# ElenaBiagi/Finito

Measured on AMD Instinct MI355X. Metric: localized k-mers/s (k=31), higher is better.
Workload: dtype u32

## Files before the change

### finito_amd/__init__.py

```python
import ctypes as C
import os
import subprocess

import numpy as np

_HERE = os.path.dirname(os.path.abspath(__file__))
_LIBPATH = os.path.join(_HERE, "libfinito_amd.so")
_LIB = None

FIN_FWD, FIN_MERGED = 0, 1
FIN_OK, FIN_EINVAL, FIN_EIO, FIN_ENODEV, FIN_ENOMEM, FIN_ELIMIT = 0, -1, -2, -3, -4, -5
X_C, X_PLANE_A, X_LCS, X_FMIN, X_USTART, X_GOFF, X_ENDS, X_CONCAT = 0, 1, 5, 6, 7, 8, 9, 10
DT_PTAB, DT_JTAB, DT_FILT, DT_SAFE, DT_RCWIN, DT_CBF, DT_FBF = range(7)


class FinitoError(RuntimeError):

    def __init__(self, code, msg):
        super().__init__("%s (code %d)" % (msg, code))
        self.code = code


def host_threads():
    n = len(os.sched_getaffinity(0)) if hasattr(os, "sched_getaffinity") else (os.cpu_count() or 1)
    for path in ("/sys/fs/cgroup/cpu.max", "/sys/fs/cgroup/cpu/cpu.cfs_quota_us"):
        try:
            txt = open(path).read().split()
            if path.endswith("cpu.max"):
# ... 948 lines not shown
        return bool(self.L.fin_index_is_disjoint(self.h))

    def seed_table(self, device=0):
        import numpy as np
        out = np.empty((self.n_nodes, 2), dtype=np.uint32)
        err = C.create_string_buffer(512)
        rc = self.L.fin_index_debug_seed_table(self.h, int(device), out.ctypes.data_as(C.c_void_p), err, 512)
        return out if rc == 0 else None

    def debug_table(self, what, device=0):
        nbytes = int(self.L.fin_index_debug_table_bytes(self.h, int(device), int(what)))
        if nbytes < 0:
            raise FinitoError(FIN_EINVAL, "debug_table: no replica on device %d, or no table %r" % (device, what))
        if nbytes == 0:
            return None
        dt = {DT_SAFE: np.uint64, DT_RCWIN: np.uint8}.get(what, np.uint32)
        out = np.zeros(nbytes // np.dtype(dt).itemsize, dtype=dt)
        err = C.create_string_buffer(512)
        _check(self.L.fin_index_debug_table(self.h, int(device), int(what), out.ctypes.data_as(C.c_void_p), out.nbytes, err, 512), err)
        return out.reshape(-1, 2) if what in (DT_PTAB, DT_JTAB) else out.reshape(-1, 4) if what in (DT_CBF, DT_FBF) else out

    def string_filter_geometry(self, device=0):
        m, lg = C.c_uint32(0), C.c_uint32(0)
        rc = self.L.fin_index_string_filter_geometry(self.h, int(device), C.byref(m), C.byref(lg))
        if rc != 0:
            raise FinitoError(rc, "string_filter_geometry: no replica on device %d" % device)
        return int(m.value), int(lg.value)

    def kmer_table_query(self, kmers, device=0):
        k = self.k
        code = {"A": 0, "C": 1, "G": 2, "T": 3}
        k0 = np.zeros(len(kmers), dtype=np.uint64); k1 = np.zeros(len(kmers), dtype=np.uint64)
        for i, s in enumerate(kmers):
            a = b = 0
            for j, ch in enumerate(s):
# ... 574 lines not shown
```

### finito_amd/csrc/fin_capi.cpp

```cpp
#include <functional>
#include <hip/hip_runtime_api.h>
#include <sched.h>

#include <algorithm>
#include <atomic>
#include <chrono>
#include <condition_variable>
#include <cstdio>
#include <cstdlib>
#include <cstring>
#include <memory>
#include <mutex>
#include <new>
#include <string>
#include <thread>
#include <vector>

#include "../../include/finito_amd.h"
#include "fin_index.hpp"
#include "fin_kernels.h"

static void set_err(char* err, size_t errlen, const std::string& msg) {
    if (err && errlen) { snprintf(err, errlen, "%s", msg.c_str()); }
}
// ... 46 lines not shown
StagePool g_stage;
bool is_page_locked(const void* p) {
    if (!p) return true;
    hipPointerAttribute_t a;
    memset(&a, 0, sizeof a);
    if (hipPointerGetAttributes(&a, p) != hipSuccess) { (void)hipGetLastError(); return false; }
    return a.type == hipMemoryTypeHost;
}
}

extern "C" {

const char* fin_version(void) { return "finito-amd 0.1 (gfx950)"; }

enum : int { O_lds_deque_limit, O_kernel, O_probe_prepass, O_ptab_t, O_jtab_t, O_write_gaps, O_overlap_prefill, O_filt_f, O_seed_anchors, O_kmer_table,
              O_defer_strand, O_fast_path, O_cbf_m, O_lean_tables, O_text_anchors, O_epoch_budget_mult, O_epoch_budget_add, O_max_batch_kmers, O_pipeline_kmers, O_pipeline_depth, O_stage_pageable, O_debug_ovf_cap, O_debug_pp_seg, O_lean_walk, O_fused_ingest, O_pp_park, O_debug_pp_park_cap, O_pp_wide_out, O_hits_combine, O_cover_probe, O_debug_depth_tile, O_ec_tag_bits, O_ec_combine, O_COUNT };
static_assert(O_COUNT <= FIN_N_OPTIONS, "fin_index::opt_val has room for every option");
struct OptDef { const char* name; int64_t def, lo, hi; };
static const OptDef OPTS[O_COUNT] = {
    {"lds_deque_limit", 16, 1, 16},
    {"kernel", 4, 0, 4},
    {"probe_prepass", 1, 0, 1},
    {"ptab_t", -1, -1, 15},
    {"jtab_t", -1, -1, 14},
    {"write_gaps", 1, 0, 1},
    {"overlap_prefill", 1, 0, 1},
    {"filt_f", -1, -1, 16},
    {"seed_anchors", 1, 0, 1},
    {"kmer_table", 1, 0, 1},
    {"defer_strand", 1, 0, 1},
    {"fast_path", 1, 0, 2},
// ... 1 lines not shown
    {"lean_tables", 2, 0, 3},
    {"text_anchors", 1, 0, 1},
    {"epoch_budget_mult", 64, 0, 64},
    {"epoch_budget_add", 4096, 1, 1 << 20},
    {"max_batch_kmers", 1ll << 30, 1, 1ll << 31},
    {"pipeline_kmers", 1ll << 26, 1, 1ll << 31},
    {"pipeline_depth", 3, 1, 8},
    {"stage_pageable", 1, 0, 1},
    {"debug_ovf_cap", 0, 0, 1ll << 31},
    {"debug_pp_seg", 0, 0, 1024},
    {"lean_walk", 1, 0, 1},
    {"fused_ingest", 1, 0, 1},
    {"pp_park", 1, 0, 1},
    {"debug_pp_park_cap", -1, -1, 1024},
    {"pp_wide_out", 1, 0, 1},
    {"hits_combine", 4, 0, 64},
    {"cover_probe", 0, 0, 1},
    {"debug_depth_tile", 0, 0, 4096},
    {"ec_tag_bits", 63, 1, 63},
    {"ec_combine", 1, 0, 1},
};
static std::atomic<int64_t> g_opt[O_COUNT];
static const bool g_opt_init = [] { for (int i = 0; i < O_COUNT; i++) g_opt[i].store(OPTS[i].def); return true; }();
static inline int64_t optv(const fin_index* x, int id) { return x && x->opt_set[id].load(std::memory_order_acquire) ? x->opt_val[id].load(std::memory_order_relaxed) : g_opt[id].load(std::memory_order_relaxed); }
static int opt_find(const char* name, int64_t value) {
    if (!name) return -1;
    for (int i = 0; i < O_COUNT; i++)
        if (!strcmp(name, OPTS[i].name)) return (value < OPTS[i].lo || value > OPTS[i].hi || (i == O_kernel && value == 1)) ? -1 : i;
    return -1;
}
// ... 142 lines not shown
int fin_index_check_against_files(const fin_index* idx, const char* sbwt_path, const char* lcs_path, char* err, size_t errlen) {
    if (!idx) { set_err(err, errlen, "null argument"); return FIN_EINVAL; }
    std::string msg; int rc = 0;
    try {
        int64_t a, b, c;
        if (sbwt_path && *sbwt_path) rc = fin_read_sbwt_file(sbwt_path, true, a, b, c, idx, msg);
        if (rc == 0 && lcs_path && *lcs_path) rc = fin_check_lcs_file(lcs_path, *idx, msg);
    } catch (const std::bad_alloc&) { rc = FIN_ENOMEM; msg = "out of memory"; }
    if (rc) set_err(err, errlen, msg);
    return rc;
}

static void free_replica(fin_index::Replica& r) {
    if (r.device >= 0) {
        (void)hipSetDevice(r.device);
        (void)hipFree(r.d_blocks); (void)hipFree(r.d_blkinfo); (void)hipFree(r.d_goff); (void)hipFree(r.d_ends); (void)hipFree(r.d_samp); (void)hipFree(r.d_concat); (void)hipFree(r.d_ptab); (void)hipFree(r.d_jtab); (void)hipFree(r.d_pos); (void)hipFree(r.d_filt); (void)hipFree(r.d_lcs8); (void)hipFree(r.d_safe); (void)hipFree(r.d_kt3); (void)hipFree(r.d_ktx); (void)hipFree(r.d_rcwin); (void)hipFree(r.d_cbf); (void)hipFree(r.d_fbf);
        r = fin_index::Replica();
    }
}
static void free_device(fin_index* x) {
    for (auto& r : x->replicas) free_replica(r);
    x->replicas.clear();
}

void fin_batch_free(fin_batch* b);
void fin_index_free(fin_index* idx) {
    if (!idx) return;
    for (auto& pb : idx->batch_pool) fin_batch_free(pb.second);
    idx->batch_pool.clear();
    free_device(idx);
    delete idx;
// ... 153 lines not shown
    d.blocks = (const FinNodeBlock*)r.d_blocks; d.blkinfo = (const FinBlockInfo*)r.d_blkinfo; d.goff = (const uint32_t*)r.d_goff;
    d.ends = (const uint32_t*)r.d_ends; d.samp = (const uint32_t*)r.d_samp; d.concat = (const uint32_t*)r.d_concat;
    d.n_nodes = (uint32_t)x->n_nodes; d.n_unitigs = (uint32_t)x->n_unitigs; d.total_len = (uint32_t)x->total_len; d.k = x->k;
    d.samp_shift = x->samp_shift; d.n_samp = (uint32_t)x->samp.size();
    for (int c = 0; c < 4; c++) d.C[c] = (uint32_t)x->C[c];
    d.C[4] = (uint32_t)x->n_nodes;
    d.lcs_t0 = x->lcs_t0;
    d.lcs8 = nullptr;
    if (!x->lcs8.empty()) {
        if ((e = up(&r.d_lcs8, x->lcs8.data(), x->lcs8.size())) != hipSuccess) {
            free_replica(r); set_err(err, errlen, std::string("uploading the LCS array: ") + hipGetErrorString(e)); return FIN_ENODEV;
        }
        d.lcs8 = (const uint8_t*)r.d_lcs8;
    }
    d.budget_mult = 64; d.budget_add = 4096;
    d.text_anchors = 0; d.defer_ok = 0; d.rcwin = nullptr;
    {
        const bool lean_req = optv(x, O_lean_tables) && optv(x, O_cbf_m) != 0 && optv(x, O_ptab_t) < 0 && x->k <= (optv(x, O_lean_tables) >= 3 ? 255u : optv(x, O_lean_tables) >= 2 ? 63u : 31u) && optv(x, O_kmer_table) && optv(x, O_seed_anchors) && optv(x, O_text_anchors) &&
                              x->total_len < FIN_POS_DUMMY && x->n_unitigs < FIN_POS_UNVERIFIED;
        int T = lean_req ? 0 : (int)optv(x, O_ptab_t);
        if (T < 0) { T = 0; while (T < 15 && T < (int)x->k && (1ull << (2 * (T + 1))) <= 16ull * x->n_nodes) T++; }
        if (T > (int)x->k) T = (int)x->k;
        d.ptab_t = 0; d.ptab = nullptr;
        if (T > 0) {
            if ((e = hipMalloc(&r.d_ptab, (sizeof(FinPrefixIval) << (2 * T)) + 16)) != hipSuccess) {
                free_replica(r); set_err(err, errlen, std::string("prefix table: ") + hipGetErrorString(e)); return FIN_ENODEV;
            }
            d.ptab_t = (uint32_t)T; d.ptab = (const FinPrefixIval*)r.d_ptab;
            const int rc = fin_launch_build_ptab(&d, r.d_ptab, T, nullptr);
            if (rc != 0 || (e = hipDeviceSynchronize()) != hipSuccess) {
                free_replica(r); set_err(err, errlen, std::string("prefix table kernel: ") + hipGetErrorString(rc ? (hipError_t)rc : e)); return FIN_ENODEV;
// ... 100 lines not shown
            uint32_t lg = 4;
            while ((8ull << lg) < x->total_len && lg < 31) lg++;
            if ((e = hipMalloc(&r.d_cbf, 16ull << lg)) != hipSuccess) {
                free_replica(r); set_err(err, errlen, std::string("canonical string filter: ") + hipGetErrorString(e)); return FIN_ENODEV;
            }
            if (r.lean && (e = hipMalloc(&r.d_fbf, 16ull << lg)) != hipSuccess) {
                free_replica(r); set_err(err, errlen, std::string("directional string filter: ") + hipGetErrorString(e)); return FIN_ENODEV;
            }
            const int rc = fin_launch_build_cbf(&d, r.d_cbf, r.d_fbf, lg, (uint32_t)m, nullptr);
            if (rc != 0 || (e = hipDeviceSynchronize()) != hipSuccess) {
                free_replica(r); set_err(err, errlen, std::string("canonical string filter kernel: ") + hipGetErrorString(rc ? (hipError_t)rc : e)); return FIN_ENODEV;
            }
            d.cbf = (const FinCbfBlock*)r.d_cbf; d.cbf_log2 = lg; d.cbf_m = (uint32_t)m; d.fbf = (const FinCbfBlock*)r.d_fbf;
        }
    }
    r.table_bytes = (r.d_ptab ? (sizeof(FinPrefixIval) << (2 * d.ptab_t)) : 0) + (r.d_jtab ? (sizeof(FinPrefixIval) << (2 * d.jtab_t)) : 0) +
                    (r.d_filt ? ((1ull << (2 * d.filt_f)) / 8) : 0) + (r.d_pos ? (x->n_nodes + 1) * sizeof(FinSeedEntry) : 0) +
                    (r.d_safe ? fin_anchor_safe_words(x->total_len) * 8 : 0) + (r.d_kt3 ? 32ull * d.kt3_buckets : 0) + (r.d_ktx ? (32ull << d.ktx_log2) : 0) +
                    (r.d_rcwin ? fin_rcwin_bytes(x->total_len) : 0) + (r.d_cbf ? (16ull << d.cbf_log2) : 0) + (r.d_fbf ? (16ull << d.cbf_log2) : 0) + (r.d_lcs8 ? x->lcs8.size() : 0);
    x->replicas.push_back(r);
    return FIN_OK;
}

int fin_index_debug_seed_table(const fin_index* x, int device, uint32_t* out, char* err, size_t errlen) {
    const fin_index::Replica* r = x ? x->replica_on(device) : nullptr;
    if (!r || !r->d_pos || !out) { set_err(err, errlen, "no seed table on that device"); return FIN_EINVAL; }
    HIPCHK(hipSetDevice(device));
    HIPCHK(hipMemcpy2D(out, 8, r->d_pos, sizeof(FinSeedEntry), 8, (size_t)x->n_nodes, hipMemcpyDeviceToHost));
    return FIN_OK;
}

static const void* debug_table_of(const fin_index* x, const fin_index::Replica& r, int what, uint64_t& bytes) {
    const FinDevIndex& d = r.dev;
    const void* p = nullptr; bytes = 0;
    switch (what) {
        case FIN_DT_PTAB: p = r.d_ptab; bytes = sizeof(FinPrefixIval) << (2 * d.ptab_t); break;
        case FIN_DT_JTAB: p = r.d_jtab; bytes = sizeof(FinPrefixIval) << (2 * d.jtab_t); break;
        case FIN_DT_FILT: p = r.d_filt; bytes = (1ull << (2 * d.filt_f)) / 8; break;
        case FIN_DT_SAFE: p = r.d_safe; bytes = (x->total_len + 63) / 64 * 8; break;
        case FIN_DT_RCWIN: p = r.d_rcwin; bytes = (x->total_len + 511) / 512; break;
        case FIN_DT_CBF: p = r.d_cbf; bytes = 16ull << d.cbf_log2; break;
        case FIN_DT_FBF: p = r.d_fbf; bytes = 16ull << d.cbf_log2; break;
        default: break;
    }
    if (!p) bytes = 0;
    return p;
}
int64_t fin_index_debug_table_bytes(const fin_index* x, int device, int what) {
    const fin_index::Replica* r = x ? x->replica_on(device) : nullptr;
    if (!r || what < FIN_DT_PTAB || what > FIN_DT_FBF) return -1;
    uint64_t bytes = 0;
    (void)debug_table_of(x, *r, what, bytes);
    return (int64_t)bytes;
}
int fin_index_debug_table(const fin_index* x, int device, int what, void* out, uint64_t out_bytes, char* err, size_t errlen) {
    if (!x || !out) { set_err(err, errlen, "null argument"); return FIN_EINVAL; }
    const fin_index::Replica* r = x->replica_on(device);
    if (!r) { set_err(err, errlen, "no replica on that device"); return FIN_EINVAL; }
    uint64_t bytes = 0;
    const void* p = debug_table_of(x, *r, what, bytes);
    if (!p) { set_err(err, errlen, "the replica on that device has no such table"); return FIN_EINVAL; }
    if (out_bytes < bytes) { set_err(err, errlen, "table buffer too small"); return FIN_EINVAL; }
    HIPCHK(hipSetDevice(device));
    HIPCHK(hipMemcpy(out, p, bytes, hipMemcpyDeviceToHost));
    return FIN_OK;
// ... 235 lines not shown
    b->dev.pp_wide_out = (uint32_t)optv(b->idx, O_pp_wide_out);
    b->dev.pp_park_cap = (uint32_t)(int32_t)optv(b->idx, O_debug_pp_park_cap);
    b->dev.lean_walk = (uint32_t)optv(b->idx, O_lean_walk);
    {
        const fin_index::Replica* rep = b->idx->replica_on(b->device);
        b->dev.text_anchors = (optv(b->idx, O_text_anchors) && rep && rep->anchors_built) ? 1u : 0u;
        b->dev.safe = rep ? rep->dev.safe : nullptr;
        b->dev.pos = (optv(b->idx, O_seed_anchors) && b->dev.text_anchors && b->d_seed && rep) ? rep->dev.pos : nullptr;
        b->dev.filt = (optv(b->idx, O_filt_f) != 0 && rep) ? rep->dev.filt : nullptr;
        const bool lean = rep && rep->lean && optv(b->idx, O_seed_anchors) && b->dev.text_anchors && b->d_seed && optv(b->idx, O_kmer_table) && rep->dev.fbf;
        b->dev.fbf = lean ? rep->dev.fbf : nullptr;
        b->dev.kt3 = (optv(b->idx, O_kmer_table) && rep && (b->dev.pos || lean)) ? rep->dev.kt3 : nullptr;
        b->dev.ktx = (b->dev.kt3 && rep) ? rep->dev.ktx : nullptr; b->dev.ktx_log2 = rep ? rep->dev.ktx_log2 : 0;
        b->dev.cbf = (rep && b->dev.kt3) ? rep->dev.cbf : nullptr;
        b->dev.fast_path = (optv(b->idx, O_fast_path) && b->dev.cbf) ? 1u : 0u;
    }
    int rc = 0;
    hipEvent_t out_ready = nullptr;
    const int opt_kernel = (int)optv(b->idx, O_kernel);
    const uint32_t lds_limit = (uint32_t)optv(b->idx, O_lds_deque_limit);
    int kern = opt_kernel;
    if (b->dev.k > FIN_FAST_K)
        kern = (opt_kernel == 4 && b->q_slots && fin_v4_writes_gaps(&b->dev, (const uint32_t*)b->d_seed)) ? 4 : 0;
    const int no_prefill = (kern == 4 && b->q_slots && optv(b->idx, O_write_gaps) && fin_v4_writes_gaps(&b->dev, (const uint32_t*)b->d_seed)) ? 1 : 0;
    {
        const fin_index::Replica* rep = b->idx->replica_on(b->device);
        b->dev.defer_ok = (kern == 4 && no_prefill && strands == FIN_MERGED && optv(b->idx, O_defer_strand) && rep && rep->anchors_built &&
                           rep->n_rc_pairs != ~0ull && (b->dev.pos || b->dev.fbf)) ? 1u : 0u;
        b->dev.rcwin = (b->dev.defer_ok && rep->d_rcwin) ? (const uint8_t*)rep->d_rcwin : nullptr;
    }
// ... 2717 lines not shown
```

### finito_amd/csrc/fin_format.h

```cpp
#pragma once
#include <stdint.h>

#define FIN_BLOCK_NODES 64
#define FIN_LCS_MASK 0x7Fu
#define FIN_USTART_BIT 0x80u
#define FIN_MAX_K 255
#define FIN_FAST_K 128

struct FinCharRec {
    uint32_t plane_lo, plane_hi;
    uint32_t base;
};
struct alignas(128) FinNodeBlock {
    uint8_t node[64];
    FinCharRec rec[4];
    uint64_t th0, th1;
};
static_assert(sizeof(FinNodeBlock) == 128, "one block = one 128-B line");
#ifdef __HIPCC__
__host__ __device__
#endif
static inline uint64_t fin_plane(const FinCharRec& r) { return r.plane_lo | ((uint64_t)r.plane_hi << 32); }

struct FinBlockInfo {
// ... 31 lines not shown
    const struct FinKt3Bucket* kt3;
    uint32_t kt3_buckets;
    const struct FinKtxSlot* ktx;
    uint32_t ktx_log2;
    const struct FinCbfBlock* cbf;
    uint32_t cbf_log2, cbf_m;
    const struct FinCbfBlock* fbf;
    uint32_t fast_path;
    uint32_t defer_ok;
    const uint8_t* rcwin;
    const uint32_t* filt;
    uint32_t filt_f;
    const uint8_t* lcs8;
    struct FinFastRec* frec;
    uint32_t text_only;
    uint32_t pp_wide_out;
    uint32_t lean_walk;
    uint32_t pp_seg;
    uint32_t pp_max_len;
    uint32_t pp_park;
    uint32_t pp_park_cap;
};
struct FinFastRec { uint32_t u, off0, meta, nk; uint64_t Es, Es2; };
struct FinDepthStat { unsigned long long sum; uint32_t max, n_at_least; };
struct FinKt3Bucket { uint32_t w[8]; };
struct FinKtxSlot { uint32_t k0_lo, k0_hi, k1_lo, k1_hi, g, claim, pad0, pad1; };
#define FIN_KT3_SLOTS 4
#define FIN_KT3_TAGMASK 0x3FFFFFFFu
#define FIN_KT3_UNVER 0x40000000u
#define FIN_KT3_EMPTY 0xFFFFFFFFFFFFFFFFull
#define FIN_KT3_LOAD_PCT 55
#ifdef __HIPCC__
__host__ __device__
#endif
static inline uint64_t fin_mix64(uint64_t x) {
    x ^= x >> 29; x *= 0xBF58476D1CE4E5B9ull; x ^= x >> 32; x *= 0x94D049BB133111EBull; x ^= x >> 29;
    return x;
// ... 49 lines not shown
```

### finito_amd/csrc/fin_index.hpp

```cpp
#pragma once
#include <cstdint>
#include <cstdlib>
#include <cstring>
#include <mutex>
#include <string>
#include <vector>

#include <atomic>

#include "fin_format.h"

#define FIN_N_OPTIONS 40

struct FinBlockArray {
    FinNodeBlock* p = nullptr;
    uint64_t n = 0;
    FinBlockArray() {}
    FinBlockArray(const FinBlockArray&) = delete;
    FinBlockArray& operator=(const FinBlockArray&) = delete;
    ~FinBlockArray() { free(p); }
    bool resize(uint64_t nb) {
        free(p); p = nullptr; n = 0;
        if (nb == 0) return true;
        void* q = nullptr;
// ... 6 lines not shown

struct fin_index {
    uint32_t k = 0;
    uint64_t n_nodes = 0, n_kmers = 0, n_unitigs = 0, total_len = 0, n_fmin = 0;
    uint64_t C[4] = {0, 0, 0, 0};
    uint32_t samp_shift = 0;
    uint32_t lcs_t0 = 0;
    FinBlockArray blocks;
    std::vector<FinBlockInfo> blkinfo;
    std::vector<uint32_t> goff, ends, samp, concat;
    std::vector<uint8_t> lcs8;
    const uint8_t* lcs8_or_null() const { return lcs8.empty() ? nullptr : lcs8.data(); }

    struct Replica {
        int device = -1;
        void* d_blocks = nullptr; void* d_blkinfo = nullptr; void* d_goff = nullptr; void* d_ends = nullptr; void* d_samp = nullptr; void* d_concat = nullptr; void* d_ptab = nullptr; void* d_jtab = nullptr; void* d_pos = nullptr; void* d_filt = nullptr; void* d_lcs8 = nullptr; void* d_safe = nullptr; void* d_kt3 = nullptr; void* d_ktx = nullptr; void* d_rcwin = nullptr; void* d_cbf = nullptr; void* d_fbf = nullptr;
        bool lean = false;
        uint64_t table_bytes = 0;
        bool anchors_built = false;
        uint64_t n_rc_pairs = 0;
        uint64_t n_unsafe = 0;
        uint64_t n_unverified = 0;
        double anchors_ms = 0;
        FinDevIndex dev{};
    };
    std::vector<Replica> replicas;
    const Replica* replica_on(int device) const {
        for (const auto& r : replicas) if (r.device == device) return &r;
        return nullptr;
    }

// ... 47 lines not shown
```

### finito_amd/csrc/fin_kernel_b.hip

```cpp
#include <hip/hip_runtime.h>
#include <stdint.h>

#include "fin_device.h"
#include "fin_kernels.h"

#define FIN_ANCH_SEG 512u

namespace {
struct BLdsDeque {
    static constexpr uint32_t CAP = 16;
    uint64_t* base; uint32_t limit;
    __device__ __forceinline__ uint64_t get(uint32_t i) const { return base[(i & (CAP - 1)) * FIN_TPB]; }
    __device__ __forceinline__ void set(uint32_t i, uint64_t v) { base[(i & (CAP - 1)) * FIN_TPB] = v; }
};
struct BGlobalDeque {
    static constexpr uint32_t CAP = 256;
    uint64_t* base; uint64_t stride; uint32_t limit;
    __device__ __forceinline__ uint64_t get(uint32_t i) const { return base[(uint64_t)(i & (CAP - 1)) * stride]; }
    __device__ __forceinline__ void set(uint32_t i, uint64_t v) { base[(uint64_t)(i & (CAP - 1)) * stride] = v; }
};

template <typename DQ>
__device__ bool anchor_segment(const FinDevIndex& ix, uint32_t s0, uint32_t s1, FinSeedEntry* pos, unsigned long long* safe, FinKt3Bucket* kt3, uint32_t kt3_buckets, DQ dq, uint32_t& n_unsafe, uint32_t* ktab_full, FinKtxSlot* ulist, uint32_t ulist_cap) {
    const uint32_t n = ix.n_nodes;
// ... 310 lines not shown
        f = (f >> 2) | (c << (2 * (m - 1u)));
        v = ((v << 2) | (3ull - c)) & mask;
        have++;
        if (have >= m && g >= s0) { cbf_insert(words, log2_blocks, f < v ? f : v); if (words_f) cbf_insert(words_f, log2_blocks, f); }
    }
}
extern "C" int fin_launch_build_cbf(const FinDevIndex* ix, void* words, void* words_f, uint32_t log2_blocks, uint32_t m, hipStream_t stream) {
    hipError_t e = hipMemsetAsync(words, 0, 16ull << log2_blocks, stream);
    if (e != hipSuccess) return (int)e;
    if (words_f && (e = hipMemsetAsync(words_f, 0, 16ull << log2_blocks, stream)) != hipSuccess) return (int)e;
    const uint64_t n_seg = ((uint64_t)ix->total_len + FIN_ANCH_SEG - 1) / FIN_ANCH_SEG;
    if (n_seg == 0 || m < 1 || m > 32) return 0;
    hipLaunchKernelGGL(fin_build_cbf_kernel, dim3((uint32_t)((n_seg + FIN_TPB - 1) / FIN_TPB)), dim3(FIN_TPB), 0, stream, *ix, (uint32_t*)words, (uint32_t*)words_f, log2_blocks, m, (uint32_t)n_seg);
    return (int)hipGetLastError();
}
```

### finito_amd/csrc/fin_kernels.h

```cpp
#pragma once
#include <hip/hip_runtime_api.h>
#include <stdint.h>

#include "fin_format.h"

#define FIN_FAST_CHUNKS 8

#ifdef __cplusplus
extern "C" {
#endif
int fin_launch_search_v0(const FinDevIndex* ix, const uint8_t* bases, const uint64_t* offs, const uint64_t* out_offs,
                         void* out, uint32_t n_reads, int strands, uint32_t lds_deque_limit, uint32_t* ovf_list, uint32_t* ovf_count,
                         uint64_t* ovf_scratch, uint32_t ovf_blocks, hipStream_t stream, hipEvent_t ev0, hipEvent_t ev1);
int fin_launch_overflow(const FinDevIndex* ix, const uint8_t* bases, const uint64_t* offs, const uint64_t* out_offs, void* out,
                        int strands, const uint32_t* ovf_list, const uint32_t* ovf_count, uint64_t* ovf_scratch, uint32_t ovf_blocks,
                        hipStream_t stream);
int fin_launch_pack_reads(const uint8_t* bases, const uint64_t* offs, const FinReadDesc* desc, void* packed, uint32_t n_reads, uint64_t n_chunks, hipStream_t stream);
int fin_launch_search_v2(const FinDevIndex* ix, const uint8_t* bases, const void* packed, const FinReadDesc* desc,
                         const uint64_t* offs, const uint64_t* out_offs, void* out, uint64_t n_kmers, uint32_t n_reads,
                         int strands, uint32_t lds_deque_limit, uint32_t* ovf_list, uint32_t* ovf_count,
                         uint32_t* work_counter, uint64_t* ovf_scratch, uint32_t ovf_blocks, uint32_t grid_blocks,
                         hipStream_t stream, hipEvent_t ev0, hipEvent_t ev1);
int fin_v2_blocks_per_cu(void);
int fin_launch_search_v3(const FinDevIndex* ix, const uint8_t* bases, const void* packed, const FinReadDesc* desc,
// ... 34 lines not shown
                         uint32_t rounds ,
                         int fused_ingest );
uint32_t fin_v4_max_rounds(void);
int fin_v4_writes_gaps(const FinDevIndex* ix, const uint32_t* seed);
int fin_probe_blocks_per_cu(void);
int fin_launch_build_ptab(const FinDevIndex* ix, void* tab, int T, hipStream_t stream);
uint64_t fin_anchor_safe_words(uint64_t total_len);
uint64_t fin_anchor_tmp_bytes(uint64_t total_len);
int fin_launch_build_anchors(const FinDevIndex* ix, struct FinSeedEntry* pos, void* safe, void* kt3, uint32_t kt3_buckets, void* tmp, uint64_t* n_unsafe, hipStream_t stream, uint64_t* n_unver);
uint32_t fin_anchor_ulist_cap(uint64_t total_len);
void* fin_anchor_ulist(void* tmp, uint64_t total_len);
int fin_launch_build_ktx(const void* ulist, uint32_t n, void* ktx, uint32_t log2, hipStream_t stream);
uint64_t fin_rcwin_bytes(uint64_t total_len);
int fin_launch_count_rc_pairs(const FinDevIndex* ix, void* tmp8, uint64_t* n_pairs, void* rcwin, hipStream_t stream);
int fin_launch_build_cbf(const FinDevIndex* ix, void* words, void* words_f, uint32_t log2_blocks, uint32_t m, hipStream_t stream);
int fin_launch_build_filter(const FinDevIndex* ix, uint32_t* filt, int F, hipStream_t stream);
int fin_launch_count_positive(const void* out, uint64_t n_pairs, unsigned long long* d_result, hipStream_t stream);
int fin_launch_set_merge(void* dst, const void* src, const uint32_t* gid, uint64_t n_pairs, int first, hipStream_t stream);
uint32_t fin_overflow_deque_cap(void);
uint32_t fin_text_blocks(uint64_t n_pairs);
uint64_t fin_text_off_words(uint64_t n_pairs);
int fin_launch_text_lengths(const void* pairs, uint64_t n_pairs, const uint64_t* out_offs, uint32_t n_reads, uint32_t* d_last_bits,
                            uint32_t* d_blk_sum, uint64_t* d_blk_off, uint64_t* d_total, hipStream_t stream);
int fin_launch_text_write(const void* pairs, uint64_t n_pairs, const uint64_t* d_blk_off, const uint32_t* d_last_bits, char* d_text, hipStream_t stream);
uint64_t fin_text3_off_words(uint64_t n_seg);
uint32_t fin_text3_seg_pairs(void);
int fin_launch_text3_lengths(const void* pairs, const uint64_t* out_offs, const void* frec, const void* seg, uint32_t n_seg, uint32_t k,
                             uint32_t* d_seg_sum, uint64_t* d_seg_off, uint64_t* d_total, unsigned long long* d_found, hipStream_t stream);
int fin_launch_text3_write(const void* pairs, const uint64_t* out_offs, const void* frec, const void* seg, uint32_t n_seg, uint32_t k,
                           const uint64_t* d_seg_off, char* d_text, hipStream_t stream);
// ... 46 lines not shown
```

### finito_amd/csrc/fin_prepass.hip

```cpp
#include <cstdio>
#include <cstring>
#include <type_traits>

#include "fin_device.h"
#include "fin_kernels.h"
#include "fin_pack.h"

#ifndef FIN_V3_PM_ADD
#define FIN_V3_PM_ADD 4
#endif
#define FIN_PP_SEG_MAX 1024

namespace {
constexpr uint32_t NONE = 0xFFFFFFFFu;

struct PpConsts {
    const char* blk_base; const FinPrefixIval* ptab; const uint32_t* filt;
    const FinCbfBlock* fbf; uint32_t fbf_mask;
    uint32_t n, C0, C1, C2, C3, C4, fmask;
    int k, PT, PM, F;
};

__device__ __forceinline__ void pp_window(const uint4& c0, const uint4& c1, int p, uint64_t& w, uint32_t& v) {
    const uint32_t j = (uint32_t)p & 31u;
// ... 339 lines not shown
        q.mw[0] |= (p >> 5) == 0u ? bit : 0u; q.mw[1] |= (p >> 5) == 1u ? bit : 0u; q.mw[2] |= (p >> 5) == 2u ? bit : 0u; q.mw[3] |= (p >> 5) == 3u ? bit : 0u;
    }
}
__device__ __forceinline__ bool cbf_known(const CbfAsk& q) {
    return (q.blk.x & q.mw[0]) == q.mw[0] && (q.blk.y & q.mw[1]) == q.mw[1] && (q.blk.z & q.mw[2]) == q.mw[2] && (q.blk.w & q.mw[3]) == q.mw[3];
}
template <typename CH>
__device__ __forceinline__ bool fast_try(const PpConsts& K, const FinDevIndex& ix, const CH& ch, uint32_t t_anchor, uint32_t r_len, uint32_t g_ans, uint64_t* lds, FastRun& res) {
    const uint32_t k = (uint32_t)K.k, m = ix.cbf_m;
    const bool put = !row_holds(ch), mir = row_mirrored(ch);
    uint32_t ls;
    const uint64_t* const arow = ask_row(ch, lds, ls);
    const uint32_t nch = (r_len + 31u) >> 5;
    if (nch > FIN_FAST_CHUNKS || g_ans < t_anchor) { PPDBG(1); return false; }
    const uint32_t gs = g_ans - t_anchor;
    uint32_t u, ustart, uend;
    {
        uint32_t idx = ix.samp[gs >> ix.samp_shift];
        uint4 e4; __builtin_memcpy(&e4, ix.ends + idx, 16);
        while (e4.w <= gs) { idx += 3u; __builtin_memcpy(&e4, ix.ends + idx, 16); }
        if (gs < e4.y) { u = idx; ustart = e4.x; uend = e4.y; }
        else if (gs < e4.z) { u = idx + 1u; ustart = e4.y; uend = e4.z; }
        else { u = idx + 2u; ustart = e4.z; uend = e4.w; }
    }
    if (gs < ustart || gs + r_len > uend) { PPDBG(2); return false; }
    const uint64_t* const text = (const uint64_t*)ix.concat;
    const uint32_t tw = gs >> 5, sh = (gs & 31u) * 2u;
    uint64_t Es = 0, Es2 = 0; uint32_t nE = 0; bool bad = false;
    auto E_at = [&](uint32_t e) -> uint32_t { return (uint32_t)((e < 4u ? Es : Es2) >> (16u * (e & 3u))) & 0xFFFFu; };
    uint64_t w0 = text[tw];
    for (uint32_t jb = 0; jb < nch; jb += 4u) {
        uint4 c[4]; uint64_t tx[4];
#pragma unroll
        for (uint32_t i = 0; i < 4u; i++) {
            const uint32_t j = jb + i < nch ? jb + i : nch - 1u;
            c[i] = ch[j]; tx[i] = text[tw + j + 1u];
        }
#pragma unroll
        for (uint32_t i = 0; i < 4u; i++) {
            const uint32_t j = jb + i;
            if (j < nch) {
                const uint64_t w1 = tx[i];
                const uint64_t tb = sh ? (w0 >> sh) | (w1 << (64u - sh)) : w0;
                w0 = w1;
                const uint64_t rb = c[i].x | ((uint64_t)c[i].y << 32);
                if (put) lds[j * FIN_TPB] = rb;
                const uint32_t nb = r_len - 32u * j < 32u ? r_len - 32u * j : 32u;
                const uint32_t vm = nb == 32u ? 0xFFFFFFFFu : (1u << nb) - 1u;
                bad = bad || (c[i].z & vm) != vm;
                const uint64_t x = rb ^ tb;
                uint64_t y = (x | (x >> 1)) & 0x5555555555555555ull;
// ... 466 lines not shown
    }
}

__global__ __launch_bounds__(FIN_TPB) void fin_pair_prepass_kernel(FinDevIndex ix, const uint4* packed, const FinReadDesc* desc, uint32_t n_reads, uint32_t seg,
                                                                   uint32_t* pass, uint32_t* seed, int defer) {
    fin_pair_prepass_body<false, false>(ix, packed, desc, n_reads, seg, pass, seed, defer, nullptr, nullptr);
}
__global__ __launch_bounds__(FIN_TPB) void fin_fast_prepass_kernel(FinDevIndex ix, const uint4* packed, const FinReadDesc* desc, uint32_t n_reads, uint32_t seg,
                                                                   uint32_t* pass, uint32_t* seed, int defer, int2* out, uint32_t* n_fast) {
    fin_pair_prepass_body<true, false>(ix, packed, desc, n_reads, seg, pass, seed, defer, out, n_fast);
}
__global__ __launch_bounds__(FIN_TPB) void fin_fast2_prepass_kernel(FinDevIndex ix, const uint4* packed, const FinReadDesc* desc, uint32_t n_reads, uint32_t seg,
                                                                    uint32_t* pass, uint32_t* seed, int defer, int2* out, uint32_t* n_fast) {
    fin_pair_prepass_body<true, true>(ix, packed, desc, n_reads, seg, pass, seed, defer, out, n_fast);
}
__global__ __launch_bounds__(FIN_TPB) void fin_fast_prepass_fused_kernel(FinDevIndex ix, uint4* packed, const FinReadDesc* desc, uint32_t n_reads, uint32_t seg,
                                                                         uint32_t* pass, uint32_t* seed, int defer, int2* out, uint32_t* n_fast, const uint8_t* bases, const uint64_t* offs,
                                                                         uint32_t rch, uint32_t cap) {
    fin_pair_prepass_body<true, false, true>(ix, packed, desc, n_reads, seg, pass, seed, defer, out, n_fast, bases, offs, packed, rch, cap);
}
__global__ __launch_bounds__(FIN_TPB) void fin_fast2_prepass_fused_kernel(FinDevIndex ix, uint4* packed, const FinReadDesc* desc, uint32_t n_reads, uint32_t seg,
                                                                          uint32_t* pass, uint32_t* seed, int defer, int2* out, uint32_t* n_fast, const uint8_t* bases, const uint64_t* offs,
                                                                          uint32_t rch, uint32_t cap) {
    fin_pair_prepass_body<true, true, true>(ix, packed, desc, n_reads, seg, pass, seed, defer, out, n_fast, bases, offs, packed, rch, cap);
}

#define FIN_PP_LDS_BUDGET 32000u
static size_t pp_fused_lds(const FinDevIndex* ix, const void* kernel, uint32_t seg, uint32_t& rch, uint32_t& cap) {
    static const size_t static_lds = [kernel] {
        hipFuncAttributes a;
        return hipFuncGetAttributes(&a, kernel) == hipSuccess && a.sharedSizeBytes ? (size_t)a.sharedSizeBytes : (size_t)(3u * 2u * FIN_PP_SEG_MAX + 64u);
    }();
    rch = ix->pp_max_len ? (ix->pp_max_len + 31u) >> 5 : FIN_FAST_CHUNKS;
    const size_t rows = (size_t)rch * FIN_TPB * 8u, slot = (size_t)rch * 8u + 4u + 2u;
    size_t c = FIN_PP_LDS_BUDGET > static_lds + rows ? (FIN_PP_LDS_BUDGET - static_lds - rows) / slot : 0u;
    if (c > seg) c = seg;
// ... 54 lines not shown
```

### include/finito_amd.h

```cpp
#ifndef FINITO_AMD_H
#define FINITO_AMD_H

#include <stddef.h>
#include <stdint.h>

#ifdef __cplusplus
extern "C" {
#endif

#define FIN_OK 0
#define FIN_EINVAL (-1)
#define FIN_EIO (-2)
#define FIN_ENODEV (-3)
#define FIN_ENOMEM (-4)
#define FIN_ELIMIT (-5)

typedef struct fin_index fin_index;
typedef struct fin_batch fin_batch;

const char* fin_version(void);

int fin_set_option(const char* name, int64_t value);
int fin_index_set_option(fin_index* idx, const char* name, int64_t value);
int fin_index_clear_option(fin_index* idx, const char* name);
// ... 35 lines not shown
int64_t fin_index_string_filter_bytes(const fin_index* idx, int device);
int64_t fin_index_replica_table_bytes(const fin_index* idx, int device);
int fin_index_first_device(const fin_index* idx);
int fin_index_is_disjoint(const fin_index* idx);
int64_t fin_index_unsafe_places(const fin_index* idx, int device);
double fin_index_anchor_build_ms(const fin_index* idx, int device);
int64_t fin_index_rc_pairs(const fin_index* idx, int device);
int fin_index_debug_seed_table(const fin_index* idx, int device, uint32_t* out, char* err, size_t errlen);
#define FIN_DT_PTAB 0
#define FIN_DT_JTAB 1
#define FIN_DT_FILT 2
#define FIN_DT_SAFE 3
#define FIN_DT_RCWIN 4
#define FIN_DT_CBF 5
#define FIN_DT_FBF 6
int64_t fin_index_debug_table_bytes(const fin_index* idx, int device, int what);
int fin_index_debug_table(const fin_index* idx, int device, int what, void* out, uint64_t out_bytes, char* err, size_t errlen);
int fin_index_string_filter_geometry(const fin_index* idx, int device, uint32_t* m, uint32_t* log2_blocks);

#define FIN_X_C 0
#define FIN_X_PLANE_A 1
#define FIN_X_LCS 5
#define FIN_X_FMIN 6
#define FIN_X_USTART 7
#define FIN_X_GOFF 8
#define FIN_X_ENDS 9
#define FIN_X_CONCAT 10
int64_t fin_index_export_size(const fin_index* idx, int what);
int fin_index_export(const fin_index* idx, int what, void* out, uint64_t out_bytes, char* err, size_t errlen);

// ... 227 lines not shown
```

Measured before the change: 201.7 billion.

## Add 128-byte text lines with inline unitig-end headers for fast-path lookup

Builds a new device table in which the concatenated text is cut into 448-base, 128-byte lines, each headed by the first unitig id, its start, and up to four unitig end offsets. The fast prepass then finds the unitig and checks that the read fits from the same cache line as the text words, avoiding the separate samp/ends lookup chain, and falls back to the old search when a line holds too many ends. It also adds a waves-per-EU occupancy hint to the two fused prepass kernels. The cost is extra device memory, a build kernel, and per-word header-skip index arithmetic in the text loop.

```diff
diff --git a/finito_amd/__init__.py b/finito_amd/__init__.py
--- a/finito_amd/__init__.py
+++ b/finito_amd/__init__.py
@@ -11,7 +11,7 @@
 FIN_FWD, FIN_MERGED = 0, 1
 FIN_OK, FIN_EINVAL, FIN_EIO, FIN_ENODEV, FIN_ENOMEM, FIN_ELIMIT = 0, -1, -2, -3, -4, -5
 X_C, X_PLANE_A, X_LCS, X_FMIN, X_USTART, X_GOFF, X_ENDS, X_CONCAT = 0, 1, 5, 6, 7, 8, 9, 10
-DT_PTAB, DT_JTAB, DT_FILT, DT_SAFE, DT_RCWIN, DT_CBF, DT_FBF = range(7)
+DT_PTAB, DT_JTAB, DT_FILT, DT_SAFE, DT_RCWIN, DT_CBF, DT_FBF, DT_TLINES = range(8)
 
 
 class FinitoError(RuntimeError):
@@ -990,11 +990,11 @@
             raise FinitoError(FIN_EINVAL, "debug_table: no replica on device %d, or no table %r" % (device, what))
         if nbytes == 0:
             return None
-        dt = {DT_SAFE: np.uint64, DT_RCWIN: np.uint8}.get(what, np.uint32)
+        dt = {DT_SAFE: np.uint64, DT_RCWIN: np.uint8, DT_TLINES: np.uint64}.get(what, np.uint32)
         out = np.zeros(nbytes // np.dtype(dt).itemsize, dtype=dt)
         err = C.create_string_buffer(512)
         _check(self.L.fin_index_debug_table(self.h, int(device), int(what), out.ctypes.data_as(C.c_void_p), out.nbytes, err, 512), err)
-        return out.reshape(-1, 2) if what in (DT_PTAB, DT_JTAB) else out.reshape(-1, 4) if what in (DT_CBF, DT_FBF) else out
+        return out.reshape(-1, 2) if what in (DT_PTAB, DT_JTAB) else out.reshape(-1, 4) if what in (DT_CBF, DT_FBF) else out.reshape(-1, 16) if what == DT_TLINES else out
 
     def string_filter_geometry(self, device=0):
         m, lg = C.c_uint32(0), C.c_uint32(0)
diff --git a/finito_amd/csrc/fin_capi.cpp b/finito_amd/csrc/fin_capi.cpp
--- a/finito_amd/csrc/fin_capi.cpp
+++ b/finito_amd/csrc/fin_capi.cpp
@@ -84,7 +84,7 @@
 const char* fin_version(void) { return "finito-amd 0.1 (gfx950)"; }
 
 enum : int { O_lds_deque_limit, O_kernel, O_probe_prepass, O_ptab_t, O_jtab_t, O_write_gaps, O_overlap_prefill, O_filt_f, O_seed_anchors, O_kmer_table,
-              O_defer_strand, O_fast_path, O_cbf_m, O_lean_tables, O_text_anchors, O_epoch_budget_mult, O_epoch_budget_add, O_max_batch_kmers, O_pipeline_kmers, O_pipeline_depth, O_stage_pageable, O_debug_ovf_cap, O_debug_pp_seg, O_lean_walk, O_fused_ingest, O_pp_park, O_debug_pp_park_cap, O_pp_wide_out, O_hits_combine, O_cover_probe, O_debug_depth_tile, O_ec_tag_bits, O_ec_combine, O_COUNT };
+              O_defer_strand, O_fast_path, O_cbf_m, O_lean_tables, O_text_anchors, O_epoch_budget_mult, O_epoch_budget_add, O_max_batch_kmers, O_pipeline_kmers, O_pipeline_depth, O_stage_pageable, O_debug_ovf_cap, O_debug_pp_seg, O_lean_walk, O_fused_ingest, O_pp_park, O_debug_pp_park_cap, O_pp_wide_out, O_text_lines, O_hits_combine, O_cover_probe, O_debug_depth_tile, O_ec_tag_bits, O_ec_combine, O_COUNT };
 static_assert(O_COUNT <= FIN_N_OPTIONS, "fin_index::opt_val has room for every option");
 struct OptDef { const char* name; int64_t def, lo, hi; };
 static const OptDef OPTS[O_COUNT] = {
@@ -116,6 +116,7 @@
     {"pp_park", 1, 0, 1},
     {"debug_pp_park_cap", -1, -1, 1024},
     {"pp_wide_out", 1, 0, 1},
+    {"text_lines", 1, 0, 1},
     {"hits_combine", 4, 0, 64},
     {"cover_probe", 0, 0, 1},
     {"debug_depth_tile", 0, 0, 4096},
@@ -288,7 +289,7 @@
 static void free_replica(fin_index::Replica& r) {
     if (r.device >= 0) {
         (void)hipSetDevice(r.device);
-        (void)hipFree(r.d_blocks); (void)hipFree(r.d_blkinfo); (void)hipFree(r.d_goff); (void)hipFree(r.d_ends); (void)hipFree(r.d_samp); (void)hipFree(r.d_concat); (void)hipFree(r.d_ptab); (void)hipFree(r.d_jtab); (void)hipFree(r.d_pos); (void)hipFree(r.d_filt); (void)hipFree(r.d_lcs8); (void)hipFree(r.d_safe); (void)hipFree(r.d_kt3); (void)hipFree(r.d_ktx); (void)hipFree(r.d_rcwin); (void)hipFree(r.d_cbf); (void)hipFree(r.d_fbf);
+        (void)hipFree(r.d_blocks); (void)hipFree(r.d_blkinfo); (void)hipFree(r.d_goff); (void)hipFree(r.d_ends); (void)hipFree(r.d_samp); (void)hipFree(r.d_concat); (void)hipFree(r.d_ptab); (void)hipFree(r.d_jtab); (void)hipFree(r.d_pos); (void)hipFree(r.d_filt); (void)hipFree(r.d_lcs8); (void)hipFree(r.d_safe); (void)hipFree(r.d_kt3); (void)hipFree(r.d_ktx); (void)hipFree(r.d_rcwin); (void)hipFree(r.d_cbf); (void)hipFree(r.d_fbf); (void)hipFree(r.d_tlines);
         r = fin_index::Replica();
     }
 }
@@ -472,7 +473,7 @@
         d.lcs8 = (const uint8_t*)r.d_lcs8;
     }
     d.budget_mult = 64; d.budget_add = 4096;
-    d.text_anchors = 0; d.defer_ok = 0; d.rcwin = nullptr;
+    d.text_anchors = 0; d.defer_ok = 0; d.rcwin = nullptr; d.tlines = nullptr;
     {
         const bool lean_req = optv(x, O_lean_tables) && optv(x, O_cbf_m) != 0 && optv(x, O_ptab_t) < 0 && x->k <= (optv(x, O_lean_tables) >= 3 ? 255u : optv(x, O_lean_tables) >= 2 ? 63u : 31u) && optv(x, O_kmer_table) && optv(x, O_seed_anchors) && optv(x, O_text_anchors) &&
                               x->total_len < FIN_POS_DUMMY && x->n_unitigs < FIN_POS_UNVERIFIED;
@@ -603,10 +604,19 @@
             d.cbf = (const FinCbfBlock*)r.d_cbf; d.cbf_log2 = lg; d.cbf_m = (uint32_t)m; d.fbf = (const FinCbfBlock*)r.d_fbf;
         }
     }
+    if (d.cbf) {
+        if ((e = hipMalloc(&r.d_tlines, fin_tlines_bytes(x->total_len))) != hipSuccess) {
+            free_replica(r); set_err(err, errlen, std::string("text lines: ") + hipGetErrorString(e)); return FIN_ENODEV;
+        }
+        const int rc = fin_launch_build_tlines(&d, r.d_tlines, x->concat.size() / 2, nullptr);
+        if (rc != 0 || (e = hipDeviceSynchronize()) != hipSuccess) {
+            free_replica(r); set_err(err, errlen, std::string("text lines kernel: ") + hipGetErrorString(rc ? (hipError_t)rc : e)); return FIN_ENODEV;
+        }
+    }
     r.table_bytes = (r.d_ptab ? (sizeof(FinPrefixIval) << (2 * d.ptab_t)) : 0) + (r.d_jtab ? (sizeof(FinPrefixIval) << (2 * d.jtab_t)) : 0) +
                     (r.d_filt ? ((1ull << (2 * d.filt_f)) / 8) : 0) + (r.d_pos ? (x->n_nodes + 1) * sizeof(FinSeedEntry) : 0) +
                     (r.d_safe ? fin_anchor_safe_words(x->total_len) * 8 : 0) + (r.d_kt3 ? 32ull * d.kt3_buckets : 0) + (r.d_ktx ? (32ull << d.ktx_log2) : 0) +
-                    (r.d_rcwin ? fin_rcwin_bytes(x->total_len) : 0) + (r.d_cbf ? (16ull << d.cbf_log2) : 0) + (r.d_fbf ? (16ull << d.cbf_log2) : 0) + (r.d_lcs8 ? x->lcs8.size() : 0);
+                    (r.d_rcwin ? fin_rcwin_bytes(x->total_len) : 0) + (r.d_cbf ? (16ull << d.cbf_log2) : 0) + (r.d_fbf ? (16ull << d.cbf_log2) : 0) + (r.d_lcs8 ? x->lcs8.size() : 0) + (r.d_tlines ? fin_tlines_bytes(x->total_len) : 0);
     x->replicas.push_back(r);
     return FIN_OK;
 }
@@ -630,6 +640,7 @@
         case FIN_DT_RCWIN: p = r.d_rcwin; bytes = (x->total_len + 511) / 512; break;
         case FIN_DT_CBF: p = r.d_cbf; bytes = 16ull << d.cbf_log2; break;
         case FIN_DT_FBF: p = r.d_fbf; bytes = 16ull << d.cbf_log2; break;
+        case FIN_DT_TLINES: p = r.d_tlines; bytes = fin_tlines_bytes(x->total_len); break;
         default: break;
     }
     if (!p) bytes = 0;
@@ -637,7 +648,7 @@
 }
 int64_t fin_index_debug_table_bytes(const fin_index* x, int device, int what) {
     const fin_index::Replica* r = x ? x->replica_on(device) : nullptr;
-    if (!r || what < FIN_DT_PTAB || what > FIN_DT_FBF) return -1;
+    if (!r || what < FIN_DT_PTAB || what > FIN_DT_TLINES) return -1;
     uint64_t bytes = 0;
     (void)debug_table_of(x, *r, what, bytes);
     return (int64_t)bytes;
@@ -903,6 +914,7 @@
         b->dev.ktx = (b->dev.kt3 && rep) ? rep->dev.ktx : nullptr; b->dev.ktx_log2 = rep ? rep->dev.ktx_log2 : 0;
         b->dev.cbf = (rep && b->dev.kt3) ? rep->dev.cbf : nullptr;
         b->dev.fast_path = (optv(b->idx, O_fast_path) && b->dev.cbf) ? 1u : 0u;
+        b->dev.tlines = (optv(b->idx, O_text_lines) && rep) ? (const uint64_t*)rep->d_tlines : nullptr;
     }
     int rc = 0;
     hipEvent_t out_ready = nullptr;
diff --git a/finito_amd/csrc/fin_format.h b/finito_amd/csrc/fin_format.h
--- a/finito_amd/csrc/fin_format.h
+++ b/finito_amd/csrc/fin_format.h
@@ -69,6 +69,7 @@
     const uint8_t* lcs8;
     struct FinFastRec* frec;
     uint32_t text_only;
+    const uint64_t* tlines;
     uint32_t pp_wide_out;
     uint32_t lean_walk;
     uint32_t pp_seg;
@@ -76,6 +77,13 @@
     uint32_t pp_park;
     uint32_t pp_park_cap;
 };
+#define FIN_TL_BASES 448u
+#define FIN_TL_WORDS 14u
+#define FIN_TL_HDR 2u
+#define FIN_TL_ENDS 4u
+#define FIN_TL_NONE 0xFFFFu
+#define FIN_TL_MORE 0xFFFEu
+static inline uint64_t fin_tlines_count(uint64_t total_len) { return (total_len + FIN_TL_BASES - 1) / FIN_TL_BASES + 2; }
 struct FinFastRec { uint32_t u, off0, meta, nk; uint64_t Es, Es2; };
 struct FinDepthStat { unsigned long long sum; uint32_t max, n_at_least; };
 struct FinKt3Bucket { uint32_t w[8]; };
diff --git a/finito_amd/csrc/fin_index.hpp b/finito_amd/csrc/fin_index.hpp
--- a/finito_amd/csrc/fin_index.hpp
+++ b/finito_amd/csrc/fin_index.hpp
@@ -44,7 +44,7 @@
 
     struct Replica {
         int device = -1;
-        void* d_blocks = nullptr; void* d_blkinfo = nullptr; void* d_goff = nullptr; void* d_ends = nullptr; void* d_samp = nullptr; void* d_concat = nullptr; void* d_ptab = nullptr; void* d_jtab = nullptr; void* d_pos = nullptr; void* d_filt = nullptr; void* d_lcs8 = nullptr; void* d_safe = nullptr; void* d_kt3 = nullptr; void* d_ktx = nullptr; void* d_rcwin = nullptr; void* d_cbf = nullptr; void* d_fbf = nullptr;
+        void* d_blocks = nullptr; void* d_blkinfo = nullptr; void* d_goff = nullptr; void* d_ends = nullptr; void* d_samp = nullptr; void* d_concat = nullptr; void* d_ptab = nullptr; void* d_jtab = nullptr; void* d_pos = nullptr; void* d_filt = nullptr; void* d_lcs8 = nullptr; void* d_safe = nullptr; void* d_kt3 = nullptr; void* d_ktx = nullptr; void* d_rcwin = nullptr; void* d_cbf = nullptr; void* d_fbf = nullptr; void* d_tlines = nullptr;
         bool lean = false;
         uint64_t table_bytes = 0;
         bool anchors_built = false;
diff --git a/finito_amd/csrc/fin_kernel_b.hip b/finito_amd/csrc/fin_kernel_b.hip
--- a/finito_amd/csrc/fin_kernel_b.hip
+++ b/finito_amd/csrc/fin_kernel_b.hip
@@ -348,3 +348,41 @@
     hipLaunchKernelGGL(fin_build_cbf_kernel, dim3((uint32_t)((n_seg + FIN_TPB - 1) / FIN_TPB)), dim3(FIN_TPB), 0, stream, *ix, (uint32_t*)words, (uint32_t*)words_f, log2_blocks, m, (uint32_t)n_seg);
     return (int)hipGetLastError();
 }
+
+__global__ __launch_bounds__(FIN_TPB) void fin_build_tlines_kernel(FinDevIndex ix, uint4* lines, uint32_t n_lines, uint32_t n_cwords) {
+    const uint32_t L = blockIdx.x * FIN_TPB + threadIdx.x;
+    if (L >= n_lines) return;
+    const uint64_t b0 = (uint64_t)L * FIN_TL_BASES, b1 = b0 + FIN_TL_BASES;
+    uint32_t u0 = ix.n_unitigs, s0 = ix.total_len;
+    uint32_t e[FIN_TL_ENDS] = {FIN_TL_NONE, FIN_TL_NONE, FIN_TL_NONE, FIN_TL_NONE};
+    if (b0 < ix.total_len) {
+        u0 = ix.samp[(uint32_t)b0 >> ix.samp_shift];
+        while (ix.ends[u0 + 1] <= (uint32_t)b0) u0++;
+        s0 = ix.ends[u0];
+        uint32_t n = 0;
+        for (uint32_t j = u0 + 1u; j <= ix.n_unitigs && ix.ends[j] < b1; j++, n++)
+            if (n < FIN_TL_ENDS) e[n] = ix.ends[j] - (uint32_t)b0;
+        if (n > FIN_TL_ENDS) e[FIN_TL_ENDS - 1u] = FIN_TL_MORE;
+    }
+    uint4* const line = lines + 8 * (size_t)L;
+    line[0] = make_uint4(u0, e[0] | (e[1] << 16), e[2] | (e[3] << 16), s0);
+    const uint64_t* const text = (const uint64_t*)ix.concat;
+    uint64_t w[FIN_TL_WORDS];
+#pragma unroll
+    for (uint32_t i = 0; i < FIN_TL_WORDS; i++) {
+        const uint64_t cw = (uint64_t)FIN_TL_WORDS * L + i, g = 32ull * cw;
+        uint64_t v = (cw < n_cwords && g < ix.total_len) ? text[cw] : 0ull;
+        if (g < ix.total_len && ix.total_len - g < 32u) v &= (1ull << (2u * (uint32_t)(ix.total_len - g))) - 1ull;
+        w[i] = v;
+    }
+#pragma unroll
+    for (uint32_t i = 0; i < FIN_TL_WORDS; i += 2)
+        line[1u + i / 2u] = make_uint4((uint32_t)w[i], (uint32_t)(w[i] >> 32), (uint32_t)w[i + 1], (uint32_t)(w[i + 1] >> 32));
+}
+extern "C" uint64_t fin_tlines_bytes(uint64_t total_len) { return 128ull * fin_tlines_count(total_len); }
+extern "C" int fin_launch_build_tlines(const FinDevIndex* ix, void* lines, uint64_t n_cwords, hipStream_t stream) {
+    const uint64_t n_lines = fin_tlines_count(ix->total_len);
+    if (n_lines > 0xFFFFFFFFull || n_cwords > 0xFFFFFFFFull) return (int)hipErrorInvalidValue;
+    hipLaunchKernelGGL(fin_build_tlines_kernel, dim3((uint32_t)((n_lines + FIN_TPB - 1) / FIN_TPB)), dim3(FIN_TPB), 0, stream, *ix, (uint4*)lines, (uint32_t)n_lines, (uint32_t)n_cwords);
+    return (int)hipGetLastError();
+}
diff --git a/finito_amd/csrc/fin_kernels.h b/finito_amd/csrc/fin_kernels.h
--- a/finito_amd/csrc/fin_kernels.h
+++ b/finito_amd/csrc/fin_kernels.h
@@ -72,6 +72,8 @@
 uint64_t fin_rcwin_bytes(uint64_t total_len);
 int fin_launch_count_rc_pairs(const FinDevIndex* ix, void* tmp8, uint64_t* n_pairs, void* rcwin, hipStream_t stream);
 int fin_launch_build_cbf(const FinDevIndex* ix, void* words, void* words_f, uint32_t log2_blocks, uint32_t m, hipStream_t stream);
+uint64_t fin_tlines_bytes(uint64_t total_len);
+int fin_launch_build_tlines(const FinDevIndex* ix, void* lines, uint64_t n_cwords, hipStream_t stream);
 int fin_launch_build_filter(const FinDevIndex* ix, uint32_t* filt, int F, hipStream_t stream);
 int fin_launch_count_positive(const void* out, uint64_t n_pairs, unsigned long long* d_result, hipStream_t stream);
 int fin_launch_set_merge(void* dst, const void* src, const uint32_t* gid, uint64_t n_pairs, int first, hipStream_t stream);
diff --git a/finito_amd/csrc/fin_prepass.hip b/finito_amd/csrc/fin_prepass.hip
--- a/finito_amd/csrc/fin_prepass.hip
+++ b/finito_amd/csrc/fin_prepass.hip
@@ -377,27 +377,49 @@
     const uint32_t nch = (r_len + 31u) >> 5;
     if (nch > FIN_FAST_CHUNKS || g_ans < t_anchor) { PPDBG(1); return false; }
     const uint32_t gs = g_ans - t_anchor;
-    uint32_t u, ustart, uend;
-    {
+    const bool lines = ix.tlines != nullptr;
+    const uint64_t* const text = lines ? ix.tlines : (const uint64_t*)ix.concat;
+    uint32_t tw = gs >> 5;
+    uint32_t u = 0, ustart = 0; bool fits = false, located = false;
+    uint64_t w0;
+    if (ix.tlines) {
+        const uint32_t L = gs / FIN_TL_BASES, o = gs - L * FIN_TL_BASES, last = o + r_len;
+        const uint4 h = *(const uint4*)(text + 16u * L);
+        const uint2 hn = *(const uint2*)(text + 16u * (last > FIN_TL_BASES ? L + 1u : L));
+        tw = 16u * L + FIN_TL_HDR + (o >> 5);
+        w0 = text[tw];
+        const uint32_t e0 = h.y & 0xFFFFu, e1 = h.y >> 16, e2 = h.z & 0xFFFFu, e3 = h.z >> 16;
+        const uint32_t c = (o >= e0 ? 1u : 0u) + (o >= e1 ? 1u : 0u) + (o >= e2 ? 1u : 0u) + (o >= e3 ? 1u : 0u);
+        const uint32_t prev = c <= 1u ? e0 : c == 2u ? e1 : c == 3u ? e2 : e3;
+        const uint32_t next = c == 0u ? e0 : c == 1u ? e1 : c == 2u ? e2 : c == 3u ? e3 : FIN_TL_NONE;
+        if (next != FIN_TL_MORE) {
+            located = true;
+            u = h.x + c; ustart = c ? gs - o + prev : h.w;
+            if (next != FIN_TL_NONE) fits = last <= next;
+            else if (last <= FIN_TL_BASES) fits = true;
+            else fits = hn.x == u && ((hn.y & 0xFFFFu) == FIN_TL_NONE || last <= FIN_TL_BASES + (hn.y & 0xFFFFu));
+        }
+    } else w0 = text[tw];
+    if (!located) {
         uint32_t idx = ix.samp[gs >> ix.samp_shift];
         uint4 e4; __builtin_memcpy(&e4, ix.ends + idx, 16);
         while (e4.w <= gs) { idx += 3u; __builtin_memcpy(&e4, ix.ends + idx, 16); }
+        uint32_t uend;
         if (gs < e4.y) { u = idx; ustart = e4.x; uend = e4.y; }
         else if (gs < e4.z) { u = idx + 1u; ustart = e4.y; uend = e4.z; }
         else { u = idx + 2u; ustart = e4.z; uend = e4.w; }
-    }
-    if (gs < ustart || gs + r_len > uend) { PPDBG(2); return false; }
-    const uint64_t* const text = (const uint64_t*)ix.concat;
-    const uint32_t tw = gs >> 5, sh = (gs & 31u) * 2u;
+        fits = gs >= ustart && gs + r_len <= uend;
+    }
+    if (!fits) { PPDBG(2); return false; }
+    const uint32_t sh = (gs & 31u) * 2u;
     uint64_t Es = 0, Es2 = 0; uint32_t nE = 0; bool bad = false;
     auto E_at = [&](uint32_t e) -> uint32_t { return (uint32_t)((e < 4u ? Es : Es2) >> (16u * (e & 3u))) & 0xFFFFu; };
-    uint64_t w0 = text[tw];
     for (uint32_t jb = 0; jb < nch; jb += 4u) {
         uint4 c[4]; uint64_t tx[4];
 #pragma unroll
         for (uint32_t i = 0; i < 4u; i++) {
             const uint32_t j = jb + i < nch ? jb + i : nch - 1u;
-            c[i] = ch[j]; tx[i] = text[tw + j + 1u];
+            c[i] = ch[j]; tx[i] = text[tw + j + 1u + (lines && (tw & 15u) + j + 1u >= 16u ? FIN_TL_HDR : 0u)];
         }
 #pragma unroll
         for (uint32_t i = 0; i < 4u; i++) {
@@ -894,12 +916,12 @@
                                                                     uint32_t* pass, uint32_t* seed, int defer, int2* out, uint32_t* n_fast) {
     fin_pair_prepass_body<true, true>(ix, packed, desc, n_reads, seg, pass, seed, defer, out, n_fast);
 }
-__global__ __launch_bounds__(FIN_TPB) void fin_fast_prepass_fused_kernel(FinDevIndex ix, uint4* packed, const FinReadDesc* desc, uint32_t n_reads, uint32_t seg,
+__global__ __launch_bounds__(FIN_TPB) __attribute__((amdgpu_waves_per_eu(5))) void fin_fast_prepass_fused_kernel(FinDevIndex ix, uint4* packed, const FinReadDesc* desc, uint32_t n_reads, uint32_t seg,
                                                                          uint32_t* pass, uint32_t* seed, int defer, int2* out, uint32_t* n_fast, const uint8_t* bases, const uint64_t* offs,
                                                                          uint32_t rch, uint32_t cap) {
     fin_pair_prepass_body<true, false, true>(ix, packed, desc, n_reads, seg, pass, seed, defer, out, n_fast, bases, offs, packed, rch, cap);
 }
-__global__ __launch_bounds__(FIN_TPB) void fin_fast2_prepass_fused_kernel(FinDevIndex ix, uint4* packed, const FinReadDesc* desc, uint32_t n_reads, uint32_t seg,
+__global__ __launch_bounds__(FIN_TPB) __attribute__((amdgpu_waves_per_eu(5))) void fin_fast2_prepass_fused_kernel(FinDevIndex ix, uint4* packed, const FinReadDesc* desc, uint32_t n_reads, uint32_t seg,
                                                                           uint32_t* pass, uint32_t* seed, int defer, int2* out, uint32_t* n_fast, const uint8_t* bases, const uint64_t* offs,
                                                                           uint32_t rch, uint32_t cap) {
     fin_pair_prepass_body<true, true, true>(ix, packed, desc, n_reads, seg, pass, seed, defer, out, n_fast, bases, offs, packed, rch, cap);
diff --git a/include/finito_amd.h b/include/finito_amd.h
--- a/include/finito_amd.h
+++ b/include/finito_amd.h
@@ -73,6 +73,7 @@
 #define FIN_DT_RCWIN 4
 #define FIN_DT_CBF 5
 #define FIN_DT_FBF 6
+#define FIN_DT_TLINES 7
 int64_t fin_index_debug_table_bytes(const fin_index* idx, int device, int what);
 int fin_index_debug_table(const fin_index* idx, int device, int what, void* out, uint64_t out_bytes, char* err, size_t errlen);
 int fin_index_string_filter_geometry(const fin_index* idx, int device, uint32_t* m, uint32_t* log2_blocks);
```

Result: no change. 203.1 billion, median of 6 (+0.7%).
